# diffqc/dqc

Measured on AMD Instinct MI355X. Metric: SCF iterations/sec (Fock build + XC grid) per GPU, cc-pVDZ 20-atom, higher is better.
Workload: dtype f64

## Files before the change

dqc_amd/csrc/grid_vxc.hip:

```cpp
#include "grid_common.hpp"

namespace dqc {

int vxc_cus_cap();

__device__ double g_vxc_det_scale = 0.0;

constexpr int VXC_WAVES = 8;

#ifndef VWS_PROD_THREADS
#define VWS_PROD_THREADS 512
#endif
constexpr int VWS_PROD = VWS_PROD_THREADS;
constexpr int VWS_NT = 512 + VWS_PROD;
constexpr int VWS2_PROD = 256, VWS2_NT = 512 + VWS2_PROD;

#ifdef VXC_TRACE
constexpr int VXC_TRACE_MAXC = 192;
__device__ long long g_vxc_trace[256 * 2 * (VXC_TRACE_MAXC + 2)];
#define VXC_TRACE_POINT(role, slot) \
    if (lane == 0 && blockIdx.x < 256 && (slot) < VXC_TRACE_MAXC + 2) g_vxc_trace[(blockIdx.x * 2 + (role)) * (VXC_TRACE_MAXC + 2) + (slot)] = wall_clock64()
#else
#define VXC_TRACE_POINT(role, slot)
#endif

constexpr int VWS_LSMAX = 256;
constexpr int VWS_GS = 4 * VWS_LSMAX;
constexpr int VWS_XS = (16 / 4) * VWS_GS;
constexpr int VWS_BUF = 2 * VWS_XS;
typedef const __attribute__((address_space(3))) double lds_cdouble_t;
constexpr int WS2_GSA = 4 * 144, WS2_GSB = 4 * 208;
constexpr int WS2_XS = 4 * WS2_GSA;
constexpr int WS2_BUF = WS2_XS + 4 * WS2_GSB;

#ifndef WS_D
#define WS_D 2
#endif
template <int MAXT, int KCH, int D = WS_D, int GSA = VWS_GS, int GSB = VWS_GS, int NTL = MAXT>
__device__ __forceinline__ void ws_chunk(const unsigned (&pa)[MAXT], const unsigned (&pb)[MAXT], v4d (&acc)[MAXT]) {
    constexpr int NS = (KCH / 4) * NTL;
    if constexpr (NTL > 0) {
        double fa[D + 1], fb[D + 1];
#pragma unroll
        for (int s = 0; s < D && s < NS; s++) {
            fa[s % (D + 1)] = *(lds_cdouble_t *)(pa[s % NTL] + (s / NTL) * GSA * 8);
            fb[s % (D + 1)] = *(lds_cdouble_t *)(pb[s % NTL] + (s / NTL) * GSB * 8);
        }
#pragma unroll
        for (int s = 0; s < NS; s++) {
            if (s + D < NS) {
                const int s2 = s + D;
                fa[s2 % (D + 1)] = *(lds_cdouble_t *)(pa[s2 % NTL] + (s2 / NTL) * GSA * 8);
                fb[s2 % (D + 1)] = *(lds_cdouble_t *)(pb[s2 % NTL] + (s2 / NTL) * GSB * 8);
            }
            __builtin_amdgcn_sched_barrier(0);
            acc[s % NTL] = mfma_f64(fa[s % (D + 1)], fb[s % (D + 1)], acc[s % NTL]);
            __builtin_amdgcn_sched_barrier(0);
        }
    }
}
struct WsTiles { int sym, T, nc, r0, c0, t0, nreal; };
__device__ __forceinline__ void ws_tile(const WsTiles &m, int u, int &li, int &lj) {
    if (m.nc) { li = u / m.nc; lj = u - li * m.nc; return; }
    if (!m.sym) { li = u / m.T; lj = u - li * m.T; return; }
    int i = 0, rem = u;
    while (rem >= m.T - i) { rem -= m.T - i; i++; }
    li = i;
    lj = i + rem;
}
template <int NTL, int KCH, int D, int GSA, int GSB, int XS, int BUF>
__device__ __forceinline__ void ws_consumer(double *lds, double *__restrict__ vmat, int ld, int nchunk, const WsTiles m, int LSA, int LSB) {
    const int lane = threadIdx.x & 63, lr = lane & 15, lk = lane >> 4;
    constexpr int NA = NTL > 0 ? NTL : 1;
    v4d acc[NA];
    unsigned pa[NA], pb[NA];
    const unsigned lds0 = (unsigned)(uintptr_t)(__attribute__((address_space(3))) double *)lds;
#pragma unroll
    for (int t = 0; t < NTL; t++) {
        acc[t] = v4d{0, 0, 0, 0};
        int li, lj;
        ws_tile(m, min(m.t0 + t, m.nreal - 1), li, lj);
        pa[t] = lds0 + 8u * (unsigned)(lk * LSA + li * 16 + lr);
        pb[t] = lds0 + 8u * (unsigned)(XS + lk * LSB + lj * 16 + lr);
    }
    __syncthreads();
    for (int c = 0; c < nchunk; c++) {
        __syncthreads();
        __syncthreads();
        if constexpr (NTL > 0) {
            ws_chunk<NA, KCH, D, GSA, GSB, NTL>(pa, pb, acc);
            const unsigned delta = (c & 1) ? (unsigned)(-BUF * 8) : (unsigned)(BUF * 8);
#pragma unroll
            for (int t = 0; t < NTL; t++) { pa[t] += delta; pb[t] += delta; }
        }
    }
#pragma unroll
    for (int t = 0; t < NTL; t++) {
        if (m.t0 + t >= m.nreal) continue;
        int li, lj;
        ws_tile(m, m.t0 + t, li, lj);
        const int ia = (m.r0 + li) * 16 + lk, ib = (m.c0 + lj) * 16 + lr;
        const double sc = (m.sym && li != lj) ? 2.0 : 1.0;
#pragma unroll
        for (int r = 0; r < 4; r++) acc_add(&vmat[(size_t)(ia + 4 * r) * ld + ib], sc * acc[t][r], g_vxc_det_scale);
    }
}
template <int MAXT, int KCH, int D, int GSA, int GSB, int XS, int BUF, int N = MAXT>
__device__ __forceinline__ void ws_consumer_n(int nt, double *lds, double *__restrict__ vmat, int ld, int nchunk, const WsTiles m,
                                              int LSA, int LSB) {
    if (nt == N) ws_consumer<N, KCH, D, GSA, GSB, XS, BUF>(lds, vmat, ld, nchunk, m, LSA, LSB);
    else if constexpr (N > 0) ws_consumer_n<MAXT, KCH, D, GSA, GSB, XS, BUF, N - 1>(nt, lds, vmat, ld, nchunk, m, LSA, LSB);
}
__device__ __forceinline__ void ws_deal(int n, int wave, int &t0, int &nt) {
    const int tbase = n / VXC_WAVES, trem = n % VXC_WAVES;
    nt = tbase + (wave < trem ? 1 : 0);
    t0 = wave * tbase + min(wave, trem);
}

template <int MAXT, int NLP, int KCH, bool GGA>
__global__ __launch_bounds__(VWS_NT, VWS_NT / 256) void vxc_ws_kernel(double *__restrict__ vmat, const double *__restrict__ ao,
                                                          int ngrid, int ld, const double *__restrict__ w,
                                                          const double *__restrict__ vrho,
                                                          const double *__restrict__ vgrad, int slab, int nsplit,
                                                          int tiles_per_split, const double *__restrict__ aob, int sym, int lda, int LS) {
    extern __shared__ __attribute__((aligned(16))) double lds[];
    static_assert(KCH == 16, "the fixed-stride chunk layout is laid out for 16-point chunks");
    constexpr int BUF = VWS_BUF;
    const int tid = threadIdx.x, wave = tid >> 6, lane = tid & 63;
    const size_t cs = (size_t)ngrid * lda;
    const int id = blockIdx.x;
    const int grp = id / (8 * nsplit), rem = id - grp * 8 * nsplit;
    const int split = rem / 8, sl = grp * 8 + (rem & 7);
    const int gs = sl * slab, ge = min(gs + slab, ngrid);
    if (gs >= ngrid) return;
    const int nchunk = (ge - gs + KCH - 1) / KCH;

    if (wave >= VXC_WAVES) {
        __builtin_amdgcn_s_setprio(3);
        constexpr int TPR = VWS_PROD / KCH;
        const int pt = tid - 512;
        const int prow = pt / TPR, pcol = pt % TPR;
        const unsigned voff0 = 8u * (unsigned)(prow * lda + pcol * 2);
        unsigned wlds = (unsigned)(uintptr_t)(__attribute__((address_space(3))) double *)lds +
                        8u * (unsigned)((prow >> 2) * VWS_GS + (prow & 3) * LS + pcol * 2);
        typedef double vd2 __attribute__((ext_vector_type(2)));
        typedef unsigned int v4u __attribute__((ext_vector_type(4)));
        typedef unsigned int v2u __attribute__((ext_vector_type(2)));
        constexpr int BUF_FLAGS = 0x00020000;
        v4u raw[NLP][GGA ? 4 : 2];
        double cf[GGA ? 4 : 1], wg = 0.0;
        auto as_d = [](unsigned lo, unsigned hi) { return __longlong_as_double((long long)(((unsigned long long)hi << 32) | lo)); };
        auto prefetch = [&](int c) {
            const int g0 = gs + c * KCH;
            const int rows = ge - g0;
            auto rsrc = [&](const double *base, size_t bytes) {
                return __builtin_amdgcn_make_buffer_rsrc((void *)base, 0, (int)bytes, BUF_FLAGS);
            };
            const v2u xw = __builtin_amdgcn_raw_buffer_load_b64(rsrc(w + g0, (size_t)rows * 8), prow * 8, 0, 0);
            wg = as_d(xw[0], xw[1]);
            const v2u xr = __builtin_amdgcn_raw_buffer_load_b64(rsrc(vrho + g0, (size_t)rows * 8), prow * 8, 0, 0);
            cf[0] = as_d(xr[0], xr[1]);
            if (GGA) {
#pragma unroll
                for (int d = 0; d < 3; d++) {
                    const v2u xg = __builtin_amdgcn_raw_buffer_load_b64(rsrc(vgrad + (size_t)d * ngrid + g0, (size_t)rows * 8), prow * 8, 0, 0);
                    cf[d + 1] = as_d(xg[0], xg[1]);
                }
            }
            const size_t nb = (size_t)rows * lda * 8;
#pragma unroll
            for (int d = 0; d < (GGA ? 4 : 1); d++) {
                const auto r = rsrc(ao + d * cs + (size_t)g0 * lda, nb);
#pragma unroll
                for (int i = 0; i < NLP; i++)
                    if ((pcol + i * TPR) * 2 < ld) raw[i][d] = __builtin_amdgcn_raw_buffer_load_b128(r, voff0 + i * TPR * 16, 0, 0);
            }
            if (!GGA && !sym) {
                const auto r = rsrc(aob + (size_t)g0 * lda, nb);
#pragma unroll
                for (int i = 0; i < NLP; i++)
                    if ((pcol + i * TPR) * 2 < ld) raw[i][1] = __builtin_amdgcn_raw_buffer_load_b128(r, voff0 + i * TPR * 16, 0, 0);
            }
        };
        auto stage = [&]() {
            cf[0] *= wg;
            if (GGA) {
#pragma unroll
                for (int d = 1; d < 4; d++) cf[d] *= 2.0 * wg;
            }
#pragma unroll
            for (int i = 0; i < NLP; i++) {
                if ((pcol + i * TPR) * 2 < ld) {
                    const v4u pb = (GGA || sym) ? raw[i][0] : raw[i][1];
                    vd2 ps = {cf[0] * as_d(pb[0], pb[1]), cf[0] * as_d(pb[2], pb[3])};
                    if (GGA) {
#pragma unroll
                        for (int d = 1; d < 4; d++) {
                            ps.x += cf[d] * as_d(raw[i][d][0], raw[i][d][1]);
                            ps.y += cf[d] * as_d(raw[i][d][2], raw[i][d][3]);
                        }
                    }
                    *(__attribute__((address_space(3))) v4u *)(wlds + i * TPR * 16) = raw[i][0];
                    *(__attribute__((address_space(3))) vd2 *)(wlds + i * TPR * 16 + VWS_XS * 8) = ps;
                }
            }
        };
        prefetch(0);
        stage();
        if (nchunk > 1) prefetch(1);
        __syncthreads();
        if (wave == VXC_WAVES) VXC_TRACE_POINT(1, 0);
        for (int c = 0; c < nchunk; c++) {
            wlds += (c & 1) ? (unsigned)(-VWS_BUF * 8) : (unsigned)(VWS_BUF * 8);
            __syncthreads();
            if (c + 1 < nchunk) stage();
            if (wave == VXC_WAVES) VXC_TRACE_POINT(1, c + 1);
            __syncthreads();
            if (c + 2 < nchunk) prefetch(c + 2);
        }
        return;
    }

    const int T = ld >> 4, ttot = sym ? T * (T + 1) / 2 : T * T;
    const int tc0 = split * tiles_per_split;
    const int tc1 = min(tc0 + tiles_per_split, ttot);
    int t0, nt;
    ws_deal(tc1 - tc0, wave, t0, nt);
    const WsTiles m{sym, T, 0, 0, 0, tc0 + t0, tc1};
    ws_consumer_n<MAXT, KCH, WS_D, VWS_GS, VWS_GS, VWS_XS, VWS_BUF>(nt, lds, vmat, ld, nchunk, m, LS, LS);
}

template <int MAXT, int NLA, int NLB, bool GGA>
__global__ __launch_bounds__(VWS2_NT, 3) void vxc_ws2_kernel(double *__restrict__ vmat, const double *__restrict__ ao,
                                                           int ngrid, int ld, const double *__restrict__ w,
                                                           const double *__restrict__ vrho,
                                                           const double *__restrict__ vgrad, int slab, int NR, int NC,
                                                           int LSA, int LSB, const double *__restrict__ aob, int lda) {
    extern __shared__ __attribute__((aligned(16))) double lds[];
    constexpr int KCH = 16;
    constexpr int BUF = WS2_BUF;
    const int tid = threadIdx.x, wave = tid >> 6, lane = tid & 63;
    const size_t cs = (size_t)ngrid * lda;
    const int T = ld >> 4, nsplit = NR * NC;
    const int id = blockIdx.x;
    const int grp = id / (8 * nsplit), rem = id - grp * 8 * nsplit;
    const int split = rem / 8, sl = grp * 8 + (rem & 7);
    const int gs = sl * slab, ge = min(gs + slab, ngrid);
    if (gs >= ngrid) return;
    const int nchunk = (ge - gs + KCH - 1) / KCH;
    const int bi = split / NC, bj = split % NC;
    const int r0 = bi * T / NR, nr = (bi + 1) * T / NR - r0;
    const int c0 = bj * T / NC, nc = (bj + 1) * T / NC - c0;
    const unsigned lds0 = (unsigned)(uintptr_t)(__attribute__((address_space(3))) double *)lds;

    if (wave >= VXC_WAVES) {
        __builtin_amdgcn_s_setprio(3);
        constexpr int TPR = VWS2_PROD / KCH;
        const int pt = tid - 512;
        const int prow = pt / TPR, pcol = pt % TPR;
        const int wa = nr * 16, wb = nc * 16;
        const unsigned voff0 = 8u * (unsigned)(prow * lda + pcol * 2);
        unsigned wla = lds0 + 8u * (unsigned)((prow >> 2) * WS2_GSA + (prow & 3) * LSA + pcol * 2);
        unsigned wlb = lds0 + 8u * (unsigned)(WS2_XS + (prow >> 2) * WS2_GSB + (prow & 3) * LSB + pcol * 2);
        typedef unsigned int v4u __attribute__((ext_vector_type(4)));
        typedef unsigned int v2u __attribute__((ext_vector_type(2)));
        typedef double vd2 __attribute__((ext_vector_type(2)));
        constexpr int BUF_FLAGS = 0x00020000;
        v4u ra[NLA], rb[NLB][GGA ? 4 : 1];
        double cf[GGA ? 4 : 1], wg = 0.0;
        auto as_d = [](unsigned lo, unsigned hi) { return __longlong_as_double((long long)(((unsigned long long)hi << 32) | lo)); };
        auto prefetch = [&](int c) {
            const int g0 = gs + c * KCH;
            const int rows = ge - g0;
            auto rsrc = [&](const double *base, size_t bytes) {
                return __builtin_amdgcn_make_buffer_rsrc((void *)base, 0, (int)bytes, BUF_FLAGS);
            };
            const v2u xw = __builtin_amdgcn_raw_buffer_load_b64(rsrc(w + g0, (size_t)rows * 8), prow * 8, 0, 0);
            wg = as_d(xw[0], xw[1]);
            const v2u xr = __builtin_amdgcn_raw_buffer_load_b64(rsrc(vrho + g0, (size_t)rows * 8), prow * 8, 0, 0);
            cf[0] = as_d(xr[0], xr[1]);
            if (GGA) {
#pragma unroll
                for (int d = 0; d < 3; d++) {
                    const v2u xg = __builtin_amdgcn_raw_buffer_load_b64(rsrc(vgrad + (size_t)d * ngrid + g0, (size_t)rows * 8), prow * 8, 0, 0);
                    cf[d + 1] = as_d(xg[0], xg[1]);
                }
            }
            const size_t nba = (size_t)rows * lda * 8 - (size_t)r0 * 128, nbb = (size_t)rows * lda * 8 - (size_t)c0 * 128;
            {
                const auto r = rsrc(ao + (size_t)g0 * lda + r0 * 16, nba);
#pragma unroll
                for (int i = 0; i < NLA; i++)
                    if ((pcol + i * TPR) * 2 < wa) ra[i] = __builtin_amdgcn_raw_buffer_load_b128(r, voff0 + i * TPR * 16, 0, 0);
            }
#pragma unroll
            for (int d = 0; d < (GGA ? 4 : 1); d++) {
                const auto r = rsrc((GGA ? ao : aob) + d * cs + (size_t)g0 * lda + c0 * 16, nbb);
#pragma unroll
                for (int i = 0; i < NLB; i++)
                    if ((pcol + i * TPR) * 2 < wb) rb[i][d] = __builtin_amdgcn_raw_buffer_load_b128(r, voff0 + i * TPR * 16, 0, 0);
            }
        };
        auto stage = [&]() {
            cf[0] *= wg;
            if (GGA) {
#pragma unroll
                for (int d = 1; d < 4; d++) cf[d] *= 2.0 * wg;
            }
#pragma unroll
            for (int i = 0; i < NLA; i++)
                if ((pcol + i * TPR) * 2 < wa) *(__attribute__((address_space(3))) v4u *)(wla + i * TPR * 16) = ra[i];
#pragma unroll
            for (int i = 0; i < NLB; i++) {
                if ((pcol + i * TPR) * 2 < wb) {
                    vd2 ps = {cf[0] * as_d(rb[i][0][0], rb[i][0][1]), cf[0] * as_d(rb[i][0][2], rb[i][0][3])};
                    if (GGA) {
#pragma unroll
                        for (int d = 1; d < 4; d++) {
                            ps.x += cf[d] * as_d(rb[i][d][0], rb[i][d][1]);
                            ps.y += cf[d] * as_d(rb[i][d][2], rb[i][d][3]);
                        }
                    }
                    *(__attribute__((address_space(3))) vd2 *)(wlb + i * TPR * 16) = ps;
                }
            }
        };
        prefetch(0);
        stage();
        if (nchunk > 1) prefetch(1);
        __syncthreads();
        for (int c = 0; c < nchunk; c++) {
            const unsigned delta = (c & 1) ? (unsigned)(-BUF * 8) : (unsigned)(BUF * 8);
            wla += delta;
            wlb += delta;
            __syncthreads();
            if (c + 1 < nchunk) stage();
            __syncthreads();
            if (c + 2 < nchunk) prefetch(c + 2);
        }
        return;
    }

    const int ntmax = ((T + NR - 1) / NR) * ((T + NC - 1) / NC);
    int t0, nt;
    ws_deal(ntmax, wave, t0, nt);
    const WsTiles m{0, T, nc, r0, c0, t0, nr * nc};
    ws_consumer_n<MAXT, KCH, 4, WS2_GSA, WS2_GSB, WS2_XS, WS2_BUF>(nt, lds, vmat, ld, nchunk, m, LSA, LSB);
}

constexpr int VWU_PROD = 256, VWU_NT = 512 + VWU_PROD;

#ifdef VWU_TRACE
constexpr int VWU_TRACE_N = 4 * 128;
__device__ long long g_vwu_trace[2 * VWU_TRACE_N];
#define VWU_STAMP(role, slot) \
    if (blockIdx.x == VWU_TRACE && (wave == 0 || wave == 8) && lane == 0 && (slot) < VWU_TRACE_N) g_vwu_trace[(role) * VWU_TRACE_N + (slot)] = wall_clock64()
#else
#define VWU_STAMP(role, slot)
#endif

template <int MAXT, int NTL, int D = 2>
__device__ __forceinline__ void wsu_chunk(const unsigned (&pi)[MAXT], const unsigned (&pj)[MAXT], v4d (&acc)[MAXT]) {
    constexpr int NS = 4 * NTL;
    double fa[D + 1], fb[D + 1];
    auto rd = [&](int s) {
        fa[s % (D + 1)] = *(lds_cdouble_t *)(pi[s % NTL] + (s / NTL) * VWS_GS * 8);
        fb[s % (D + 1)] = *(lds_cdouble_t *)(pj[s % NTL] + ((s / NTL) * VWS_GS + VWS_XS) * 8);
    };
#pragma unroll
    for (int s = 0; s < D && s < NS; s++) rd(s);
#pragma unroll
    for (int s = 0; s < NS; s++) {
        if (s + D < NS) rd(s + D);
        __builtin_amdgcn_sched_barrier(0);
        acc[s % NTL] = mfma_f64(fa[s % (D + 1)], fb[s % (D + 1)], acc[s % NTL]);
        __builtin_amdgcn_sched_barrier(0);
    }
}

template <int MAXT, int N = MAXT>
__device__ __forceinline__ void wsu_chunk_n(int nt, const unsigned (&pi)[MAXT], const unsigned (&pj)[MAXT], v4d (&acc)[MAXT]) {
    if constexpr (N == 0) return;
    else if (nt == N) wsu_chunk<MAXT, N>(pi, pj, acc);
    else wsu_chunk_n<MAXT, N - 1>(nt, pi, pj, acc);
}

template <int NLP, bool GGA>
DQC_DEV void vwu_producer(double *lds, const double *__restrict__ ao, int ngrid, int ld, const double *__restrict__ w,
                          const double *__restrict__ vrho, const double *__restrict__ vgrad, int gs, int ge, int nchunk,
                          int lda, int LS) {
    constexpr int KCH = 16;
    const int tid = threadIdx.x, wave = tid >> 6, lane = tid & 63;
    (void)wave; (void)lane;
    const size_t cs = (size_t)ngrid * lda;
    __builtin_amdgcn_s_setprio(3);
    constexpr int TPR = VWU_PROD / KCH;
    const int pt = tid - 512;
    const int prow = pt / TPR, pcol = pt % TPR;
    const unsigned voff0 = 8u * (unsigned)(prow * lda + pcol * 2);
    unsigned wlds = (unsigned)(uintptr_t)(__attribute__((address_space(3))) double *)lds +
                    8u * (unsigned)((prow >> 2) * VWS_GS + (prow & 3) * LS + pcol * 2);
    typedef double vd2 __attribute__((ext_vector_type(2)));
    typedef unsigned int v4u __attribute__((ext_vector_type(4)));
    typedef unsigned int v2u __attribute__((ext_vector_type(2)));
    constexpr int BUF_FLAGS = 0x00020000;
    v4u raw[NLP][GGA ? 4 : 1];
    double cf[GGA ? 4 : 1], wg = 0.0;
    auto as_d = [](unsigned lo, unsigned hi) { return __longlong_as_double((long long)(((unsigned long long)hi << 32) | lo)); };
    auto prefetch = [&](int c) {
        const int g0 = gs + c * KCH;
        const int rows = ge - g0;
        auto rsrc = [&](const double *base, size_t bytes) {
            return __builtin_amdgcn_make_buffer_rsrc((void *)base, 0, (int)bytes, BUF_FLAGS);
        };
        const v2u xw = __builtin_amdgcn_raw_buffer_load_b64(rsrc(w + g0, (size_t)rows * 8), prow * 8, 0, 0);
        wg = as_d(xw[0], xw[1]);
        const v2u xr = __builtin_amdgcn_raw_buffer_load_b64(rsrc(vrho + g0, (size_t)rows * 8), prow * 8, 0, 0);
        cf[0] = as_d(xr[0], xr[1]);
        if (GGA) {
#pragma unroll
            for (int d = 0; d < 3; d++) {
                const v2u xg = __builtin_amdgcn_raw_buffer_load_b64(rsrc(vgrad + (size_t)d * ngrid + g0, (size_t)rows * 8), prow * 8, 0, 0);
                cf[d + 1] = as_d(xg[0], xg[1]);
            }
        }
        const size_t nb = (size_t)rows * lda * 8;
#pragma unroll
        for (int d = 0; d < (GGA ? 4 : 1); d++) {
            const auto r = rsrc(ao + d * cs + (size_t)g0 * lda, nb);
#pragma unroll
            for (int i = 0; i < NLP; i++)
                if ((pcol + i * TPR) * 2 < ld) raw[i][d] = __builtin_amdgcn_raw_buffer_load_b128(r, voff0 + i * TPR * 16, 0, 0);
        }
    };
    auto stage = [&]() {
        cf[0] *= wg;
        if (GGA) {
#pragma unroll
            for (int d = 1; d < 4; d++) cf[d] *= 2.0 * wg;
        }
#pragma unroll
        for (int i = 0; i < NLP; i++) {
            if ((pcol + i * TPR) * 2 < ld) {
                vd2 ps = {cf[0] * as_d(raw[i][0][0], raw[i][0][1]), cf[0] * as_d(raw[i][0][2], raw[i][0][3])};
                if (GGA) {
#pragma unroll
                    for (int d = 1; d < 4; d++) {
                        ps.x += cf[d] * as_d(raw[i][d][0], raw[i][d][1]);
                        ps.y += cf[d] * as_d(raw[i][d][2], raw[i][d][3]);
                    }
                }
                *(__attribute__((address_space(3))) v4u *)(wlds + i * TPR * 16) = raw[i][0];
                *(__attribute__((address_space(3))) vd2 *)(wlds + i * TPR * 16 + VWS_XS * 8) = ps;
            }
        }
    };
    prefetch(0);
    stage();
    if (nchunk > 1) prefetch(1);
    __syncthreads();
#ifdef VWU_TRACE
    if (blockIdx.x == VWU_TRACE && tid == 512) { g_vwu_trace[VWU_TRACE_N - 4] = clock64(); g_vwu_trace[VWU_TRACE_N - 3] = wall_clock64(); }
#endif
    for (int c = 0; c < nchunk; c++) {
        wlds += (c & 1) ? (unsigned)(-VWS_BUF * 8) : (unsigned)(VWS_BUF * 8);
        __syncthreads();
#ifdef VWU_TRACE_CHUNKS
        VWU_STAMP(1, 4 * c);
        asm volatile("s_waitcnt vmcnt(0)" ::: "memory");
        VWU_STAMP(1, 4 * c + 1);
#endif
#ifndef VWU_EXP_NOSTAGE
        if (c + 1 < nchunk) stage();
#endif
        __syncthreads();
#ifndef VWU_EXP_NOLOAD
        if (c + 2 < nchunk) prefetch(c + 2);
#endif
    }
#ifdef VWU_TRACE
    if (blockIdx.x == VWU_TRACE && tid == 512) { g_vwu_trace[VWU_TRACE_N - 2] = clock64(); g_vwu_trace[VWU_TRACE_N - 1] = wall_clock64(); }
#endif
}

template <int MAXT, int NLP>
__global__ __launch_bounds__(VWU_NT, 3) void vxc_wsu_kernel(double *__restrict__ vmat, const double *__restrict__ ao, int ngrid,
                                                           int ld, const double *__restrict__ w, const double *__restrict__ vrho,
                                                           const double *__restrict__ vgrad, int slab, int lda, int LS) {
    extern __shared__ __attribute__((aligned(16))) double lds[];
    constexpr int KCH = 16;
    const int tid = threadIdx.x, wave = tid >> 6, lane = tid & 63;
    const int gs = blockIdx.x * slab, ge = min(gs + slab, ngrid);
    if (gs >= ngrid) return;
    const int nchunk = (ge - gs + KCH - 1) / KCH;

    if (wave >= VXC_WAVES) {
        vwu_producer<NLP, false>(lds, ao, ngrid, ld, w, vrho, vgrad, gs, ge, nchunk, lda, LS);
        return;
    }

    const int lr = lane & 15, lk = lane >> 4;
    const int T = ld >> 4, ttot = T * (T + 1) / 2;
    auto tile_ij = [&](int u, int &ti, int &tj) {
        int i = 0, rem = u;
        while (rem >= T - i) { rem -= T - i; i++; }
        ti = i;
        tj = i + rem;
    };
    const int tbase = ttot / VXC_WAVES, trem = ttot % VXC_WAVES;
    const int nt = tbase + (wave < trem ? 1 : 0);
    const int t0 = wave * tbase + min(wave, trem);
    v4d acc[MAXT];
    unsigned pi[MAXT], pj[MAXT];
    const unsigned lds0 = (unsigned)(uintptr_t)(__attribute__((address_space(3))) double *)lds;
#pragma unroll
    for (int t = 0; t < MAXT; t++) {
        acc[t] = v4d{0, 0, 0, 0};
        int ti, tj;
        tile_ij(min(t0 + min(t, max(nt - 1, 0)), ttot - 1), ti, tj);
        pi[t] = lds0 + 8u * (unsigned)(lk * LS + ti * 16 + lr);
        pj[t] = lds0 + 8u * (unsigned)(lk * LS + tj * 16 + lr);
    }
    __syncthreads();
    for (int c = 0; c < nchunk; c++) {
#ifdef VWU_TRACE_CONS
        VWU_STAMP(0, 4 * c);
#endif
        __syncthreads();
        __syncthreads();
#ifdef VWU_TRACE_CONS
        VWU_STAMP(0, 4 * c + 1);
#endif
#ifndef VWU_EXP_NOMFMA
        wsu_chunk_n<MAXT>(nt, pi, pj, acc);
#endif
        const unsigned delta = (c & 1) ? (unsigned)(-VWS_BUF * 8) : (unsigned)(VWS_BUF * 8);
#pragma unroll
        for (int t = 0; t < MAXT; t++) { pi[t] += delta; pj[t] += delta; }
    }
#pragma unroll
    for (int t = 0; t < MAXT; t++) {
        if (t < nt) {
            int ti, tj;
            tile_ij(t0 + t, ti, tj);
            const int ia = ti * 16 + lk, ib = tj * 16 + lr;
            const double sc = ti != tj ? 2.0 : 1.0;
#ifdef VWU_EXP_NOEPI
            if (acc[t][0] != 1.2345e300) continue;
#endif
#pragma unroll
            for (int r = 0; r < 4; r++) acc_add(&vmat[(size_t)(ia + 4 * r) * ld + ib], sc * acc[t][r], g_vxc_det_scale);
        }
    }
}

constexpr int wsd_ls(int T) { return ((16 * T) & 31) == 16 ? 16 * T : 16 * T + 16; }

template <int T>
struct WsdDeal {
    int no[VXC_WAVES], nd[VXC_WAVES], o0[VXC_WAVES], d0[VXC_WAVES];
    constexpr WsdDeal() : no{}, nd{}, o0{}, d0{} {
        const int noff = T * (T - 1) / 2;
        int cost[4] = {0, 0, 0, 0};
        for (int w = 0; w < VXC_WAVES; w++) {
            no[w] = noff / VXC_WAVES + (w < noff % VXC_WAVES ? 1 : 0);
            cost[w & 3] += 2 * no[w];
        }
        for (int d = 0; d < T; d++) {
            int q = 0;
            for (int r = 1; r < 4; r++)
                if (cost[r] < cost[q]) q = r;
            const int w = no[q] + nd[q] <= no[q + 4] + nd[q + 4] ? q : q + 4;
            nd[w]++;
            cost[q]++;
        }
        for (int w = 1; w < VXC_WAVES; w++) {
            o0[w] = o0[w - 1] + no[w - 1];
            d0[w] = d0[w - 1] + nd[w - 1];
        }
    }
    constexpr int max_tiles() const {
        int m = 0;
        for (int w = 0; w < VXC_WAVES; w++) m = no[w] + nd[w] > m ? no[w] + nd[w] : m;
        return m;
    }
};

template <int NO, int ND, int D = 2>
DQC_DEV void wsd_chunk(const unsigned (&pi)[NO + ND], const unsigned (&pj)[NO + ND], v4d (&acc)[NO + ND]) {
    constexpr int PER = 2 * NO + ND, NS = 4 * PER;
    double fa[D + 1], fb[D + 1];
    auto rd = [&](int s) {
        const int kk = s / PER, u = s % PER;
        const int t = u < 2 * NO ? u / 2 : NO + (u - 2 * NO), h = u < 2 * NO ? u % 2 : 0;
        fa[s % (D + 1)] = *(lds_cdouble_t *)(pi[t] + (kk * VWS_GS + (h ? VWS_XS : 0)) * 8);
        fb[s % (D + 1)] = *(lds_cdouble_t *)(pj[t] + (kk * VWS_GS + (h ? 0 : VWS_XS)) * 8);
    };
#pragma unroll
    for (int s = 0; s < D && s < NS; s++) rd(s);
#pragma unroll
    for (int s = 0; s < NS; s++) {
        if (s + D < NS) rd(s + D);
        __builtin_amdgcn_sched_barrier(0);
        const int u = s % PER;
        const int t = u < 2 * NO ? u / 2 : NO + (u - 2 * NO);
        acc[t] = mfma_f64(fa[s % (D + 1)], fb[s % (D + 1)], acc[t]);
        __builtin_amdgcn_sched_barrier(0);
    }
}

template <int T, int NO, int ND>
DQC_DEV void wsd_consumer(double *lds, double *__restrict__ vmat, int nchunk, int o0, int d0) {
    constexpr int NT = NO + ND, LS = wsd_ls(T);
    const int lane = threadIdx.x & 63, lr = lane & 15, lk = lane >> 4;
    auto tile_ij = [&](int t, int &ti, int &tj) {
        if (t >= NO) { ti = tj = d0 + (t - NO); return; }
        int i = 0, rem = o0 + t;
        while (rem >= T - 1 - i) { rem -= T - 1 - i; i++; }
        ti = i;
        tj = i + 1 + rem;
    };
    v4d acc[NT];
    unsigned pi[NT], pj[NT];
    const unsigned lds0 = (unsigned)(uintptr_t)(__attribute__((address_space(3))) double *)lds;
#pragma unroll
    for (int t = 0; t < NT; t++) {
        acc[t] = v4d{0, 0, 0, 0};
        int ti, tj;
        tile_ij(t, ti, tj);
        pi[t] = lds0 + 8u * (unsigned)(lk * LS + ti * 16 + lr);
        pj[t] = lds0 + 8u * (unsigned)(lk * LS + tj * 16 + lr);
    }
    __syncthreads();
    for (int c = 0; c < nchunk; c++) {
        __syncthreads();
        __syncthreads();
        wsd_chunk<NO, ND>(pi, pj, acc);
        const unsigned delta = (c & 1) ? (unsigned)(-VWS_BUF * 8) : (unsigned)(VWS_BUF * 8);
#pragma unroll
        for (int t = 0; t < NT; t++) { pi[t] += delta; pj[t] += delta; }
    }
#pragma unroll
    for (int t = 0; t < NT; t++) {
        int ti, tj;
        tile_ij(t, ti, tj);
        const int ia = ti * 16 + lk, ib = tj * 16 + lr;
#pragma unroll
        for (int r = 0; r < 4; r++) acc_add(&vmat[(size_t)(ia + 4 * r) * (16 * T) + ib], acc[t][r], g_vxc_det_scale);
    }
}

template <int T, int NLP>
__global__ __launch_bounds__(VWU_NT, 3) void vxc_wsd_kernel(double *__restrict__ vmat, const double *__restrict__ ao, int ngrid,
                                                           const double *__restrict__ w, const double *__restrict__ vrho,
                                                           const double *__restrict__ vgrad, int slab, int lda) {
    extern __shared__ __attribute__((aligned(16))) double lds[];
    constexpr int KCH = 16, ld = 16 * T;
    constexpr WsdDeal<T> DL{};
    static_assert(DL.max_tiles() <= 12, "more than 12 accumulator tiles per wave");
    const int wave = threadIdx.x >> 6;
    const int gs = blockIdx.x * slab, ge = min(gs + slab, ngrid);
    if (gs >= ngrid) return;
    const int nchunk = (ge - gs + KCH - 1) / KCH;
    if (wave >= VXC_WAVES) {
        vwu_producer<NLP, true>(lds, ao, ngrid, ld, w, vrho, vgrad, gs, ge, nchunk, lda, wsd_ls(T));
        return;
    }
#define DQC_WSD_CASE(W) case W: wsd_consumer<T, DL.no[W], DL.nd[W]>(lds, vmat, nchunk, DL.o0[W], DL.d0[W]); break;
    switch (wave) {
        DQC_WSD_CASE(0) DQC_WSD_CASE(1) DQC_WSD_CASE(2) DQC_WSD_CASE(3)
        DQC_WSD_CASE(4) DQC_WSD_CASE(5) DQC_WSD_CASE(6) DQC_WSD_CASE(7)
    }
#undef DQC_WSD_CASE
}



__global__ void symmetrize_kernel(double *m, int ld, int nao) {
    const int i = blockIdx.y * 16 + threadIdx.y, j = blockIdx.x * 16 + threadIdx.x;
    const double sc = g_vxc_det_scale;
    if (i < ld && j < i) {
        const double v = i < nao ? 0.5 * (det_value(m[(size_t)i * ld + j], sc) + det_value(m[(size_t)j * ld + i], sc)) : 0.0;
        m[(size_t)i * ld + j] = v;
        m[(size_t)j * ld + i] = v;
    } else if (i < ld && j == i) {
        if (i >= nao) m[(size_t)i * ld + i] = 0.0;
        else if (sc != 0.0) m[(size_t)i * ld + i] = det_value(m[(size_t)i * ld + i], sc);
    }
}

static int sync_vxc_det_scale() {
    static double current[64];
    int dev = 0;
    if (hipGetDevice(&dev) != hipSuccess || dev < 0 || dev >= 64) return 0;
    const double want = deterministic_mode() ? 140737488355328.0 : 0.0;
    if (current[dev] != want) {
        DQC_HIP(hipMemcpyToSymbol(HIP_SYMBOL(g_vxc_det_scale), &want, sizeof(double)));
        current[dev] = want;
    }
    return 0;
}

template <int MAXT, int NLP, int KCH, bool GGA>
static void launch_vxc_ws_inst(dim3 grid, size_t shmem, hipStream_t st, double *vmat, const double *ao, int ngrid, int ld,
                               const double *w, const double *vrho, const double *vgrad, int slab, int nsplit, int tps,
                               const double *aob, int sym, int lda, int LS) {
    auto kern = vxc_ws_kernel<MAXT, NLP, KCH, GGA>;
    (void)hipFuncSetAttribute((const void *)kern, hipFuncAttributeMaxDynamicSharedMemorySize, (int)shmem);
    hipLaunchKernelGGL(kern, grid, dim3(VWS_NT), shmem, st, vmat, ao, ngrid, ld, w, vrho, vgrad, slab, nsplit, tps, aob, sym, lda, LS);
}

template <bool GGA>
static int launch_vxc_ws(int maxt, int nlp, dim3 grid, size_t shmem, hipStream_t st, double *vmat,
                         const double *ao, int ngrid, int ld, const double *w, const double *vrho, const double *vgrad,
                         int slab, int nsplit, int tps, const double *aob, int sym, int lda, int LS) {
#define DQC_VWS_CASE(N, L)                                                                                          \
    if (maxt == N && nlp == L) {                                                                                    \
        launch_vxc_ws_inst<N, L, 16, GGA>(grid, shmem, st, vmat, ao, ngrid, ld, w, vrho, vgrad, slab, nsplit, tps, aob, sym, lda, LS); \
        return 0;                                                                                                   \
    }
    DQC_VWS_CASE(2, 1) DQC_VWS_CASE(4, 1) DQC_VWS_CASE(6, 1) DQC_VWS_CASE(8, 1) DQC_VWS_CASE(11, 1)
    DQC_VWS_CASE(2, 2) DQC_VWS_CASE(4, 2) DQC_VWS_CASE(6, 2) DQC_VWS_CASE(8, 2) DQC_VWS_CASE(11, 2)
    DQC_VWS_CASE(2, 4) DQC_VWS_CASE(4, 4) DQC_VWS_CASE(6, 4) DQC_VWS_CASE(8, 4) DQC_VWS_CASE(11, 4)
#undef DQC_VWS_CASE
    set_error("vxc_ws: internal dispatch error");
    return DQC_EINVAL;
}

template <int MAXT>
static void launch_vxc_wsu(dim3 grid, size_t shmem, hipStream_t st, double *vmat, const double *ao, int ngrid, int ld,
                                const double *w, const double *vrho, const double *vgrad, int slab, int lda, int LS) {
    auto kern = vxc_wsu_kernel<MAXT, 7>;
    (void)hipFuncSetAttribute((const void *)kern, hipFuncAttributeMaxDynamicSharedMemorySize, (int)shmem);
    hipLaunchKernelGGL(kern, grid, dim3(VWU_NT), shmem, st, vmat, ao, ngrid, ld, w, vrho, vgrad, slab, lda, LS);
}

template <int T>
static void launch_vxc_wsd(dim3 grid, size_t shmem, hipStream_t st, double *vmat, const double *ao, int ngrid, const double *w,
                           const double *vrho, const double *vgrad, int slab, int lda) {
    auto kern = vxc_wsd_kernel<T, 7>;
    (void)hipFuncSetAttribute((const void *)kern, hipFuncAttributeMaxDynamicSharedMemorySize, (int)shmem);
    hipLaunchKernelGGL(kern, grid, dim3(VWU_NT), shmem, st, vmat, ao, ngrid, w, vrho, vgrad, slab, lda);
}

template <int MAXT, int NLA, int NLB, bool GGA>
static void launch_vxc_ws2_inst(dim3 grid, size_t shmem, hipStream_t st, double *vmat, const double *ao, int ngrid, int ld,
                                const double *w, const double *vrho, const double *vgrad, int slab, int NR, int NC, int LSA,
                                int LSB, const double *aob, int lda) {
    auto kern = vxc_ws2_kernel<MAXT, NLA, NLB, GGA>;
    (void)hipFuncSetAttribute((const void *)kern, hipFuncAttributeMaxDynamicSharedMemorySize, (int)shmem);
    hipLaunchKernelGGL(kern, grid, dim3(VWS2_NT), shmem, st, vmat, ao, ngrid, ld, w, vrho, vgrad, slab, NR, NC, LSA, LSB, aob, lda);
}

template <bool GGA>
static int launch_vxc_ws2(int maxt, int nla, int nlb, dim3 grid, size_t shmem, hipStream_t st, double *vmat, const double *ao,
                          int ngrid, int ld, const double *w, const double *vrho, const double *vgrad, int slab, int NR,
                          int NC, int LSA, int LSB, const double *aob, int lda) {
#define DQC_VW2_CASE(N, A, B)                                                                                        \
    if (maxt == N && nla == A && nlb == B) {                                                                          \
        launch_vxc_ws2_inst<N, A, B, GGA>(grid, shmem, st, vmat, ao, ngrid, ld, w, vrho, vgrad, slab, NR, NC, LSA, LSB, aob, lda); \
        return 0;                                                                                                     \
    }
    DQC_VW2_CASE(8, 4, 4) DQC_VW2_CASE(8, 4, 6) DQC_VW2_CASE(11, 4, 4) DQC_VW2_CASE(11, 4, 6)
    DQC_VW2_CASE(8, 5, 4) DQC_VW2_CASE(8, 5, 6) DQC_VW2_CASE(11, 5, 4) DQC_VW2_CASE(11, 5, 6)
#undef DQC_VW2_CASE
    set_error("vxc_ws2: internal dispatch error");
    return DQC_EINVAL;
}

}

extern "C" {

static int grid_vxc_impl(double *d_vmat, const double *d_ao, const double *d_aob, int ncomp, int ngrid, int nao,
                         const double *d_w, const double *d_vrho, const double *d_vgrad, void *stream, bool raw = false) {
    using namespace dqc;
    hipStream_t st = (hipStream_t)stream;
    const bool gga = d_vgrad != nullptr;
    if (gga && ncomp < 4) { set_error("dqc_grid_vxc: vgrad given but ao has < 4 components"); return DQC_EINVAL; }
    const int ld = dqc_padded_nao(nao), lda = dqc_ao_stride(nao), T = ld / 16;
    auto pad16 = [](int w_) { return (w_ & 31) == 16 ? w_ : w_ + 16; };
    const int LS = pad16(ld);
    if (sync_vxc_det_scale()) return DQC_EHIP;
    DQC_HIP(hipMemsetAsync(d_vmat, 0, sizeof(double) * (size_t)ld * ld, st));
    if (ngrid <= 0) return DQC_OK;
    const bool ws_shape = LS <= VWS_LSMAX, one_operand = d_aob == d_ao;
    const bool sym = ws_shape && !gga && one_operand;
    const int ttot = sym ? T * (T + 1) / 2 : T * T;
    auto slabs = [&](int nslab, int mult, int &slab) {
        slab = (ngrid + nslab - 1) / nslab;
        slab = (slab + 15) / 16 * 16;
        return ((ngrid + slab - 1) / slab + mult - 1) / mult * mult;
    };
    int rc = 0, slab = 0;
    if (ttot > 2 * 11 * VXC_WAVES) {
        int NR = (T + 8) / 9, NC = 1;
        {
            const int nrm = (T + NR - 1) / NR;
            while ((T + NC - 1) / NC > 12 || nrm * ((T + NC - 1) / NC) > 11 * VXC_WAVES) NC++;
            const char *e1 = getenv("DQC_WS2_NR"), *e2 = getenv("DQC_WS2_NC");
            if (e1 && atoi(e1) > 0) NR = atoi(e1);
            if (e2 && atoi(e2) > 0) NC = atoi(e2);
        }
        const int nrmax = (T + NR - 1) / NR, ncmax = (T + NC - 1) / NC;
        if (nrmax > 9 || ncmax > 12 || nrmax * ncmax > 11 * VXC_WAVES) { set_error("vxc_ws2: rectangle outside the kernel's limits"); return DQC_EINVAL; }
        const int need = (nrmax * ncmax + VXC_WAVES - 1) / VXC_WAVES;
        const int maxt = need <= 8 ? 8 : 11;
        const int LSA = pad16(nrmax * 16), LSB = pad16(ncmax * 16);
        if (LSA > 144 || LSB > 208) { set_error("vxc_ws2: internal layout error"); return DQC_EINVAL; }
        const int nla = nrmax <= 8 ? 4 : 5, nlb = (ncmax * 8 + 15) / 16 <= 4 ? 4 : 6;
        const int nsplit = NR * NC;
        static const int target_blocks = [] { const char *e = getenv("DQC_VXC_BLOCKS"); return e && atoi(e) > 0 ? atoi(e) : 512; }();
        const int nslab = slabs(std::max(8, std::min(target_blocks / nsplit, std::max(ngrid / 1024, 512 / nsplit)) / 8 * 8), 8, slab);
        const size_t shmem = sizeof(double) * 2 * WS2_BUF;
        const dim3 grid(nslab * nsplit);
        rc = gga ? launch_vxc_ws2<true>(maxt, nla, nlb, grid, shmem, st, d_vmat, d_ao, ngrid, ld, d_w, d_vrho, d_vgrad, slab, NR, NC, LSA, LSB, d_aob, lda)
                 : launch_vxc_ws2<false>(maxt, nla, nlb, grid, shmem, st, d_vmat, d_ao, ngrid, ld, d_w, d_vrho, d_vgrad, slab, NR, NC, LSA, LSB, d_aob, lda);
    } else if (ws_shape && T >= 10 && T * (T + 1) / 2 <= 12 * VXC_WAVES && one_operand) {
        int ncu = stream_cus(st);
        if (vxc_cus_cap() > 0) ncu = std::max(8, std::min(ncu, vxc_cus_cap()));
        const dim3 grid(slabs(ncu, 1, slab));
        const size_t shmem = sizeof(double) * 2 * VWS_BUF;
        if (gga) {
            if (T == 13) launch_vxc_wsd<13>(grid, shmem, st, d_vmat, d_ao, ngrid, d_w, d_vrho, d_vgrad, slab, lda);
            else if (T == 12) launch_vxc_wsd<12>(grid, shmem, st, d_vmat, d_ao, ngrid, d_w, d_vrho, d_vgrad, slab, lda);
            else if (T == 11) launch_vxc_wsd<11>(grid, shmem, st, d_vmat, d_ao, ngrid, d_w, d_vrho, d_vgrad, slab, lda);
            else launch_vxc_wsd<10>(grid, shmem, st, d_vmat, d_ao, ngrid, d_w, d_vrho, d_vgrad, slab, lda);
        } else if ((T * (T + 1) / 2 + VXC_WAVES - 1) / VXC_WAVES <= 9) {
            launch_vxc_wsu<9>(grid, shmem, st, d_vmat, d_ao, ngrid, ld, d_w, d_vrho, d_vgrad, slab, lda, LS);
        } else {
            launch_vxc_wsu<12>(grid, shmem, st, d_vmat, d_ao, ngrid, ld, d_w, d_vrho, d_vgrad, slab, lda, LS);
        }
    } else if (ws_shape) {
        static const int sizes_ws[] = {2, 4, 6, 8, 11};
        const int cap = 11 * VXC_WAVES;
        const int nsplit = (ttot + cap - 1) / cap;
        const int tps = (ttot + nsplit - 1) / nsplit;
        const int need = (tps + VXC_WAVES - 1) / VXC_WAVES;
        int maxt = 11;
        for (int q = 0; q < 5; q++)
            if (sizes_ws[q] >= need) { maxt = sizes_ws[q]; break; }
        const int tprp = VWS_PROD / 16;
        const int nlpneed = (ld / 2 + tprp - 1) / tprp;
        const int nlp = nlpneed <= 1 ? 1 : (nlpneed <= 2 ? 2 : 4);
        const int nslab = slabs(std::max(8, (stream_cus(st) / nsplit) / 8 * 8), 8, slab);
        const size_t shmem = sizeof(double) * 2 * VWS_BUF;
        const dim3 grid(nslab * nsplit);
        rc = gga ? launch_vxc_ws<true>(maxt, nlp, grid, shmem, st, d_vmat, d_ao, ngrid, ld, d_w, d_vrho, d_vgrad, slab, nsplit, tps, d_aob, 0, lda, LS)
                 : launch_vxc_ws<false>(maxt, nlp, grid, shmem, st, d_vmat, d_ao, ngrid, ld, d_w, d_vrho, d_vgrad, slab, nsplit, tps, d_aob, sym ? 1 : 0, lda, LS);
    } else {
        set_error("dqc_grid_vxc: internal dispatch error (no kernel family for this shape)");
        return DQC_EINVAL;
    }
    if (rc) return rc;
    DQC_CHECK_LAUNCH();
    if (!raw) hipLaunchKernelGGL(symmetrize_kernel, dim3((ld + 15) / 16, (ld + 15) / 16), dim3(16, 16), 0, st, d_vmat, ld, nao);
    DQC_CHECK_LAUNCH();
    return DQC_OK;
}

int dqc_grid_vxc(double *d_vmat, const double *d_ao, int ncomp, int ngrid, int nao, const double *d_w,
                 const double *d_vrho, const double *d_vgrad, void *stream) {
    return grid_vxc_impl(d_vmat, d_ao, d_ao, ncomp, ngrid, nao, d_w, d_vrho, d_vgrad, stream);
}

int dqc_grid_vxc_raw(double *d_vmat, const double *d_ao, int ncomp, int ngrid, int nao, const double *d_w, const double *d_vrho,
                     const double *d_vgrad, double *h_scale, void *stream) {
    if (h_scale) *h_scale = dqc::deterministic_mode() ? 140737488355328.0 : 0.0;
    return grid_vxc_impl(d_vmat, d_ao, d_ao, ncomp, ngrid, nao, d_w, d_vrho, d_vgrad, stream, true);
}

int dqc_grid_vxc_pair(double *d_vmat, const double *d_ao_a, const double *d_ao_b, int ngrid, int nao, const double *d_w,
                      const double *d_v, void *stream) {
    return grid_vxc_impl(d_vmat, d_ao_a, d_ao_b, 1, ngrid, nao, d_w, d_v, nullptr, stream);
}

#ifdef VWU_TRACE
int dqc_debug_vwu_trace(long long *host_out) {
    return (int)hipMemcpyFromSymbol(host_out, HIP_SYMBOL(dqc::g_vwu_trace), sizeof(long long) * 2 * dqc::VWU_TRACE_N);
}
#endif


}
```

Baseline: 793.6.

## Assign WSD tiles to waves via fixed ownership table to reuse LDS fragments

Replaces the contiguous off-diagonal/diagonal tile dealing in the symmetric VXC consumer with a precomputed per-T ownership table. Each wave now loads only the distinct row fragments it needs (at most 7) into registers once per k-group and reuses them across its tiles, instead of two LDS reads per MFMA. Reads for the next k-group are interleaved with MFMAs through compile-time slices. Static asserts check full coverage, MFMA balance across SIMDs and the fragment count. In exchange it uses more registers for fragments and restricts T to 10..13.

```diff
diff --git a/dqc_amd/csrc/grid_vxc.hip b/dqc_amd/csrc/grid_vxc.hip
--- a/dqc_amd/csrc/grid_vxc.hip
+++ b/dqc_amd/csrc/grid_vxc.hip
@@ -1,3 +1,5 @@
+#include <utility>
+
 #include "grid_common.hpp"
 
 namespace dqc {
@@ -556,98 +558,160 @@
 
 constexpr int wsd_ls(int T) { return ((16 * T) & 31) == 16 ? 16 * T : 16 * T + 16; }
 
+constexpr int WSD_TMIN = 10, WSD_TMAX = 13, WSD_NTRI = WSD_TMAX * (WSD_TMAX + 1) / 2;
+constexpr int WSD_MAXTILES = 12;
+constexpr int WSD_MAXU = 7;
+constexpr signed char WSD_OWNER[WSD_TMAX - WSD_TMIN + 1][WSD_NTRI] = {
+    {7, 0, 3, 3, 2, 2, 7, 2, 0, 0, 4, 0, 1, 4, 1, 4, 2, 0, 4, 3, 3, 3, 5, 5, 7, 0, 7, 1, 3, 1, 6, 6, 6, 1, 3, 5, 4, 2, 5, 4, 2, 5, 2, 5, 1, 6, 7, 6, 7, 6, 6, 7, 5, 4, 1},
+    {5, 0, 6, 0, 5, 3, 6, 0, 5, 5, 3, 0, 7, 7, 4, 2, 2, 0, 4, 7, 2, 6, 7, 6, 3, 6, 3, 6, 7, 3, 1, 1, 1, 0, 0, 1, 7, 1, 5, 1, 6, 4, 4, 5, 1, 1, 2, 3, 1, 2, 3, 0, 0, 6, 2, 2, 3, 4, 7, 4, 5, 5, 4, 5, 2, 3},
+    {4, 0, 0, 4, 7, 4, 7, 0, 1, 1, 0, 1, 3, 0, 6, 6, 6, 2, 0, 3, 2, 2, 3, 2, 5, 5, 0, 5, 5, 1, 1, 2, 1, 5, 6, 4, 5, 4, 6, 5, 4, 4, 5, 7, 3, 6, 3, 7, 3, 3, 7, 7, 6, 6, 7, 0, 4, 2, 5, 3, 2, 2, 7, 5, 6, 5, 0, 4, 1, 1, 3, 1, 2, 2, 7, 2, 3, 4},
+    {0, 2, 0, 0, 1, 1, 2, 2, 6, 0, 6, 2, 6, 4, 3, 3, 4, 5, 5, 2, 3, 4, 4, 4, 2, 6, 7, 3, 7, 3, 7, 3, 0, 6, 7, 7, 0, 4, 7, 3, 7, 0, 0, 4, 0, 7, 3, 1, 3, 1, 3, 1, 4, 4, 1, 5, 5, 1, 5, 5, 5, 7, 1, 3, 2, 5, 5, 5, 2, 2, 7, 6, 1, 6, 7, 6, 3, 0, 6, 0, 6, 1, 5, 0, 1, 4, 4, 6, 2, 2, 6},
+};
+constexpr int WSD_NU[WSD_TMAX - WSD_TMIN + 1][VXC_WAVES] = {
+    {5, 4, 5, 4, 5, 5, 4, 5}, {5, 5, 5, 5, 5, 4, 5, 5}, {6, 5, 5, 6, 6, 6, 6, 6}, {6, 6, 6, 6, 6, 6, 6, 6}};
+
 template <int T>
 struct WsdDeal {
-    int no[VXC_WAVES], nd[VXC_WAVES], o0[VXC_WAVES], d0[VXC_WAVES];
-    constexpr WsdDeal() : no{}, nd{}, o0{}, d0{} {
-        const int noff = T * (T - 1) / 2;
-        int cost[4] = {0, 0, 0, 0};
+    int nt[VXC_WAVES], no[VXC_WAVES], nu[VXC_WAVES], nm[VXC_WAVES];
+    int ti[VXC_WAVES][WSD_NTRI], tj[VXC_WAVES][WSD_NTRI];
+    int si[VXC_WAVES][WSD_NTRI], sj[VXC_WAVES][WSD_NTRI];
+    int u[VXC_WAVES][WSD_TMAX];
+    int owned;
+    constexpr WsdDeal() : nt{}, no{}, nu{}, nm{}, ti{}, tj{}, si{}, sj{}, u{}, owned(0) {
+        for (int pass = 0; pass < 2; pass++)
+            for (int i = 0, k = 0; i < T; i++)
+                for (int j = i; j < T; j++, k++) {
+                    const int w = WSD_OWNER[T - WSD_TMIN][k];
+                    if (w < 0 || w >= VXC_WAVES || (i == j) != (pass == 1)) continue;
+                    ti[w][nt[w]] = i;
+                    tj[w][nt[w]] = j;
+                    nt[w]++;
+                    no[w] += i != j;
+                    nm[w] += i != j ? 2 : 1;
+                    owned++;
+                }
         for (int w = 0; w < VXC_WAVES; w++) {
-            no[w] = noff / VXC_WAVES + (w < noff % VXC_WAVES ? 1 : 0);
-            cost[w & 3] += 2 * no[w];
-        }
-        for (int d = 0; d < T; d++) {
-            int q = 0;
-            for (int r = 1; r < 4; r++)
-                if (cost[r] < cost[q]) q = r;
-            const int w = no[q] + nd[q] <= no[q + 4] + nd[q + 4] ? q : q + 4;
-            nd[w]++;
-            cost[q]++;
-        }
-        for (int w = 1; w < VXC_WAVES; w++) {
-            o0[w] = o0[w - 1] + no[w - 1];
-            d0[w] = d0[w - 1] + nd[w - 1];
+            for (int x = 0; x < T; x++) {
+                bool used = false;
+                for (int t = 0; t < nt[w]; t++) used = used || ti[w][t] == x || tj[w][t] == x;
+                if (used) u[w][nu[w]++] = x;
+            }
+            for (int t = 0; t < nt[w]; t++)
+                for (int s = 0; s < nu[w]; s++) {
+                    if (u[w][s] == ti[w][t]) si[w][t] = s;
+                    if (u[w][s] == tj[w][t]) sj[w][t] = s;
+                }
         }
     }
     constexpr int max_tiles() const {
         int m = 0;
-        for (int w = 0; w < VXC_WAVES; w++) m = no[w] + nd[w] > m ? no[w] + nd[w] : m;
+        for (int w = 0; w < VXC_WAVES; w++) m = nt[w] > m ? nt[w] : m;
         return m;
     }
+    constexpr int simd_spread() const {
+        int lo = nm[0] + nm[4], hi = lo;
+        for (int q = 1; q < 4; q++) {
+            const int c = nm[q] + nm[q + 4];
+            lo = c < lo ? c : lo;
+            hi = c > hi ? c : hi;
+        }
+        return hi - lo;
+    }
+    constexpr int mfmas() const {
+        int m = 0;
+        for (int w = 0; w < VXC_WAVES; w++) m += nm[w];
+        return m;
+    }
+    constexpr bool nu_as_stated() const {
+        for (int w = 0; w < VXC_WAVES; w++)
+            if (nu[w] != WSD_NU[T - WSD_TMIN][w] || nu[w] > WSD_MAXU) return false;
+        return true;
+    }
 };
-
-template <int NO, int ND, int D = 2>
-DQC_DEV void wsd_chunk(const unsigned (&pi)[NO + ND], const unsigned (&pj)[NO + ND], v4d (&acc)[NO + ND]) {
-    constexpr int PER = 2 * NO + ND, NS = 4 * PER;
-    double fa[D + 1], fb[D + 1];
-    auto rd = [&](int s) {
-        const int kk = s / PER, u = s % PER;
-        const int t = u < 2 * NO ? u / 2 : NO + (u - 2 * NO), h = u < 2 * NO ? u % 2 : 0;
-        fa[s % (D + 1)] = *(lds_cdouble_t *)(pi[t] + (kk * VWS_GS + (h ? VWS_XS : 0)) * 8);
-        fb[s % (D + 1)] = *(lds_cdouble_t *)(pj[t] + (kk * VWS_GS + (h ? 0 : VWS_XS)) * 8);
-    };
-#pragma unroll
-    for (int s = 0; s < D && s < NS; s++) rd(s);
-#pragma unroll
-    for (int s = 0; s < NS; s++) {
-        if (s + D < NS) rd(s + D);
+template <int T>
+struct WsdDealOf {
+    static constexpr WsdDeal<T> v{};
+    static_assert(v.owned == T * (T + 1) / 2, "an upper-triangle tile without an owner wave");
+    static_assert(v.mfmas() == T * T, "T^2 MFMAs per k-group");
+    static_assert(v.max_tiles() <= WSD_MAXTILES, "more than 12 accumulator tiles per wave");
+    static_assert(v.simd_spread() <= 1, "the SIMDs' MFMA counts differ by more than one");
+    static_assert(v.nu_as_stated(), "per-wave fragment count |U| is not the stated one (or above 7)");
+};
+
+template <int T, int W, int S, int X, int KK>
+constexpr int wsd_frag_off() { return (WsdDealOf<T>::v.u[W][S] * 16 + KK * VWS_GS + X * VWS_XS) * 8; }
+
+template <int T, int W>
+struct WsdChunk {
+    static constexpr int NT = WsdDealOf<T>::v.nt[W], NO = WsdDealOf<T>::v.no[W], NU = WsdDealOf<T>::v.nu[W];
+    static constexpr int NM = WsdDealOf<T>::v.nm[W], NR = 2 * NU;
+    typedef double Frags[2][2 * WSD_MAXU];
+
+    template <int KK, int R>
+    static DQC_DEV void read(unsigned base, Frags &f) {
+        f[KK & 1][R] = *(lds_cdouble_t *)(base + wsd_frag_off<T, W, R / 2, R % 2, KK>());
+    }
+    template <int KK, int... R>
+    static DQC_DEV void read_all(unsigned base, Frags &f, std::integer_sequence<int, R...>) {
+        (read<KK, R>(base, f), ...);
+    }
+    static constexpr int NMR = NM > 2 ? NM - 2 : 1;
+    template <int KK, int M, int R = M * NR / NMR>
+    static DQC_DEV void read_slice(unsigned base, Frags &f) {
+        if constexpr (M < NMR && R < (M + 1) * NR / NMR) {
+            read<KK, R>(base, f);
+            read_slice<KK, M, R + 1>(base, f);
+        }
+    }
+    template <int KK, int M>
+    static DQC_DEV void step(unsigned base, Frags &f, v4d (&acc)[NT]) {
+        constexpr int t = M < NO ? M : M - NO, h = M >= NO && M < 2 * NO ? 1 : 0;
+        constexpr int a = 2 * WsdDealOf<T>::v.si[W][t] + h, b = 2 * WsdDealOf<T>::v.sj[W][t] + (1 - h);
+        if constexpr (KK < 3) read_slice<KK + 1, M>(base, f);
         __builtin_amdgcn_sched_barrier(0);
-        const int u = s % PER;
-        const int t = u < 2 * NO ? u / 2 : NO + (u - 2 * NO);
-        acc[t] = mfma_f64(fa[s % (D + 1)], fb[s % (D + 1)], acc[t]);
+        acc[t] = mfma_f64(f[KK & 1][a], f[KK & 1][b], acc[t]);
         __builtin_amdgcn_sched_barrier(0);
     }
-}
-
-template <int T, int NO, int ND>
-DQC_DEV void wsd_consumer(double *lds, double *__restrict__ vmat, int nchunk, int o0, int d0) {
-    constexpr int NT = NO + ND, LS = wsd_ls(T);
+    template <int KK, int... M>
+    static DQC_DEV void kgroup(unsigned base, Frags &f, v4d (&acc)[NT], std::integer_sequence<int, M...>) {
+        (step<KK, M>(base, f, acc), ...);
+    }
+    static DQC_DEV void run(unsigned base, v4d (&acc)[NT]) {
+        Frags f;
+        read_all<0>(base, f, std::make_integer_sequence<int, NR>{});
+        kgroup<0>(base, f, acc, std::make_integer_sequence<int, NM>{});
+        kgroup<1>(base, f, acc, std::make_integer_sequence<int, NM>{});
+        kgroup<2>(base, f, acc, std::make_integer_sequence<int, NM>{});
+        kgroup<3>(base, f, acc, std::make_integer_sequence<int, NM>{});
+    }
+    template <int... TL>
+    static DQC_DEV void store(double *__restrict__ vmat, const v4d (&acc)[NT], int lr, int lk, std::integer_sequence<int, TL...>) {
+        auto one = [&](int t, int ti, int tj) {
+            const int ia = ti * 16 + lk, ib = tj * 16 + lr;
+#pragma unroll
+            for (int r = 0; r < 4; r++) acc_add(&vmat[(size_t)(ia + 4 * r) * (16 * T) + ib], acc[t][r], g_vxc_det_scale);
+        };
+        (one(TL, WsdDealOf<T>::v.ti[W][TL], WsdDealOf<T>::v.tj[W][TL]), ...);
+    }
+};
+
+template <int T, int W>
+DQC_DEV void wsd_consumer(double *lds, double *__restrict__ vmat, int nchunk) {
+    typedef WsdChunk<T, W> CH;
+    constexpr int LS = wsd_ls(T);
     const int lane = threadIdx.x & 63, lr = lane & 15, lk = lane >> 4;
-    auto tile_ij = [&](int t, int &ti, int &tj) {
-        if (t >= NO) { ti = tj = d0 + (t - NO); return; }
-        int i = 0, rem = o0 + t;
-        while (rem >= T - 1 - i) { rem -= T - 1 - i; i++; }
-        ti = i;
-        tj = i + 1 + rem;
-    };
-    v4d acc[NT];
-    unsigned pi[NT], pj[NT];
-    const unsigned lds0 = (unsigned)(uintptr_t)(__attribute__((address_space(3))) double *)lds;
-#pragma unroll
-    for (int t = 0; t < NT; t++) {
-        acc[t] = v4d{0, 0, 0, 0};
-        int ti, tj;
-        tile_ij(t, ti, tj);
-        pi[t] = lds0 + 8u * (unsigned)(lk * LS + ti * 16 + lr);
-        pj[t] = lds0 + 8u * (unsigned)(lk * LS + tj * 16 + lr);
-    }
+    v4d acc[CH::NT];
+#pragma unroll
+    for (int t = 0; t < CH::NT; t++) acc[t] = v4d{0, 0, 0, 0};
+    unsigned base = (unsigned)(uintptr_t)(__attribute__((address_space(3))) double *)lds + 8u * (unsigned)(lk * LS + lr);
     __syncthreads();
     for (int c = 0; c < nchunk; c++) {
         __syncthreads();
         __syncthreads();
-        wsd_chunk<NO, ND>(pi, pj, acc);
-        const unsigned delta = (c & 1) ? (unsigned)(-VWS_BUF * 8) : (unsigned)(VWS_BUF * 8);
-#pragma unroll
-        for (int t = 0; t < NT; t++) { pi[t] += delta; pj[t] += delta; }
-    }
-#pragma unroll
-    for (int t = 0; t < NT; t++) {
-        int ti, tj;
-        tile_ij(t, ti, tj);
-        const int ia = ti * 16 + lk, ib = tj * 16 + lr;
-#pragma unroll
-        for (int r = 0; r < 4; r++) acc_add(&vmat[(size_t)(ia + 4 * r) * (16 * T) + ib], acc[t][r], g_vxc_det_scale);
-    }
+        CH::run(base, acc);
+        base += (c & 1) ? (unsigned)(-VWS_BUF * 8) : (unsigned)(VWS_BUF * 8);
+    }
+    CH::store(vmat, acc, lr, lk, std::make_integer_sequence<int, CH::NT>{});
 }
 
 template <int T, int NLP>
@@ -656,8 +720,7 @@
                                                            const double *__restrict__ vgrad, int slab, int lda) {
     extern __shared__ __attribute__((aligned(16))) double lds[];
     constexpr int KCH = 16, ld = 16 * T;
-    constexpr WsdDeal<T> DL{};
-    static_assert(DL.max_tiles() <= 12, "more than 12 accumulator tiles per wave");
+    static_assert(T >= WSD_TMIN && T <= WSD_TMAX, "no ownership table for this T");
     const int wave = threadIdx.x >> 6;
     const int gs = blockIdx.x * slab, ge = min(gs + slab, ngrid);
     if (gs >= ngrid) return;
@@ -666,15 +729,13 @@
         vwu_producer<NLP, true>(lds, ao, ngrid, ld, w, vrho, vgrad, gs, ge, nchunk, lda, wsd_ls(T));
         return;
     }
-#define DQC_WSD_CASE(W) case W: wsd_consumer<T, DL.no[W], DL.nd[W]>(lds, vmat, nchunk, DL.o0[W], DL.d0[W]); break;
+#define DQC_WSD_CASE(W) case W: wsd_consumer<T, W>(lds, vmat, nchunk); break;
     switch (wave) {
         DQC_WSD_CASE(0) DQC_WSD_CASE(1) DQC_WSD_CASE(2) DQC_WSD_CASE(3)
         DQC_WSD_CASE(4) DQC_WSD_CASE(5) DQC_WSD_CASE(6) DQC_WSD_CASE(7)
     }
 #undef DQC_WSD_CASE
 }
-
-
 
 __global__ void symmetrize_kernel(double *m, int ld, int nao) {
     const int i = blockIdx.y * 16 + threadIdx.y, j = blockIdx.x * 16 + threadIdx.x;
```

Measured after the change: 802.1, median of 6. 1.1% higher.
